# Coloquinte/sleekit

Measured on AMD Instinct MI355X. Metric: Mweights/sec quantized (GPTQ 3-bit, 4096x4096 layer), higher is better.
Workload: dtype f64; 1 GPU; 8 layers 4096x4096, 8-level uniform codebook (GPTQ 3-bit), act_order=diag, damp=0.01, local-search moves=0, layer error included; distinct_inputs=8, allocator_settle_steps=15, gpu_max_hw_queues=4

## Files before the change

sleekit_amd/csrc/api.hip:

```cpp
#include "mfma32.h"
#include "mfma64.h"

namespace slk {

__global__ __launch_bounds__(256) void k_probe_f64(double *sink, int iters) {
    double4_t c0 = {0, 0, 0, 0}, c1 = c0, c2 = c0, c3 = c0;
    const double a = 1.0 + threadIdx.x * 1e-3, b = 1.0 - threadIdx.x * 1e-3;
    for (int i = 0; i < iters; ++i) {
        c0 = __builtin_amdgcn_mfma_f64_16x16x4f64(a, b, c0, 0, 0, 0);
        c1 = __builtin_amdgcn_mfma_f64_16x16x4f64(b, a, c1, 0, 0, 0);
        c2 = __builtin_amdgcn_mfma_f64_16x16x4f64(a, a, c2, 0, 0, 0);
        c3 = __builtin_amdgcn_mfma_f64_16x16x4f64(b, b, c3, 0, 0, 0);
    }
    const double4_t s = c0 + c1 + c2 + c3;
    if (s[0] + s[1] + s[2] + s[3] == 12345.678) sink[0] = s[0];
}

template <int NACC>
__global__ __launch_bounds__(256) void k_probe_f64_n(double *sink, int iters) {
    double4_t c[NACC];
    double a[NACC], b[NACC];
#pragma unroll
    for (int i = 0; i < NACC; ++i) {
        c[i] = (double4_t){0, 0, 0, 0};
// ... 67 lines not shown
}

using namespace slk;

extern "C" {

int slk_probe_chain(double *out, int iters, int mode, slk_stream_t stream) {
    SLK_REQUIRE(out && iters > 0, "bad arguments");
    hipStream_t s = as_stream(stream);
    SLK_RUN("probe_chain", 0, 0, s, k_probe_chain<<<1, 64, 0, s>>>(out, iters, mode));
    return SLK_OK;
}

size_t slk_workspace_bytes(int R, int n) {
    if (R < 0 || n <= 0) return 0;
    const size_t ld = (size_t)slk_factor_ld(n);
    const size_t rn = (size_t)(R > 0 ? R : 1) * (size_t)n;
    size_t factor = 2 * ld * ld * sizeof(double) + 2 * (ld / 64) * sizeof(int);
    size_t loop = 2 * rn * sizeof(float) + (size_t)n * sizeof(int) + 64 * sizeof(float) + 5 * 256;
    size_t search = rn * sizeof(float) + (size_t)(R + n) * sizeof(float) + (size_t)R * ((n + 127) / 128) * sizeof(float) + 4096;
    size_t error = 6 * (rn + 128 * (size_t)n) + 6 * (size_t)n * n + 4 * (size_t)R * ((n + 127) / 128) * sizeof(float) + 8192;
    size_t prep = 64 * sizeof(float) + (size_t)n * (sizeof(double) + 1);
    search += error;
    size_t m = factor;
    if (loop > m) m = loop;
    if (search > m) m = search;
    if (error > m) m = error;
    if (prep > m) m = prep;
    return m + (1u << 16);
}

size_t slk_workspace_bytes_batch(int batch, int rows_per_layer, int n) {
    if (batch < 1 || batch > 64 || rows_per_layer < 0 || n <= 0 || (long long)batch * rows_per_layer > 0x7fffffffLL) return 0;
    return slk_workspace_bytes(batch * rows_per_layer, n) + (size_t)(batch - 1) * 6 * (size_t)n * n +
           (size_t)batch * n * (sizeof(int) + sizeof(float)) + (size_t)(batch - 1) * 64 * sizeof(float) +
           4096;
}

int slk_probe_mfma_f64(double *sink, int blocks, int iters, slk_stream_t stream) {
    SLK_REQUIRE(sink && blocks > 0 && iters > 0, "bad arguments");
    hipStream_t s = as_stream(stream);
    SLK_RUN("probe_mfma_f64", 4.0 * 2048 * 4 * iters * blocks, 0, s, k_probe_f64<<<blocks, 256, 0, s>>>(sink, iters));
    return SLK_OK;
}

int slk_probe_mfma_f64_acc(double *sink, int blocks, int iters, int nacc, slk_stream_t stream) {
    SLK_REQUIRE(sink && blocks > 0 && iters > 0 && (nacc == 1 || nacc == 2 || nacc == 4 || nacc == 8 || nacc == 16), "bad arguments");
    hipStream_t s = as_stream(stream);
    if (nacc == 1)
        SLK_RUN("probe_mfma_f64", 1.0 * 2048 * 4 * iters * blocks, 0, s, k_probe_f64_n<1><<<blocks, 256, 0, s>>>(sink, iters));
    else if (nacc == 2)
        SLK_RUN("probe_mfma_f64", 2.0 * 2048 * 4 * iters * blocks, 0, s, k_probe_f64_n<2><<<blocks, 256, 0, s>>>(sink, iters));
    else if (nacc == 4)
        SLK_RUN("probe_mfma_f64", 4.0 * 2048 * 4 * iters * blocks, 0, s, k_probe_f64_n<4><<<blocks, 256, 0, s>>>(sink, iters));
    else if (nacc == 8)
        SLK_RUN("probe_mfma_f64", 8.0 * 2048 * 4 * iters * blocks, 0, s, k_probe_f64_n<8><<<blocks, 256, 0, s>>>(sink, iters));
    else
        SLK_RUN("probe_mfma_f64", 16.0 * 2048 * 4 * iters * blocks, 0, s, k_probe_f64_n<16><<<blocks, 256, 0, s>>>(sink, iters));
    return SLK_OK;
}

int slk_probe_mfma_f32(float *sink, int blocks, int iters, slk_stream_t stream) {
    SLK_REQUIRE(sink && blocks > 0 && iters > 0, "bad arguments");
    hipStream_t s = as_stream(stream);
    SLK_RUN("probe_mfma_f32", 4.0 * 4096 * 4 * iters * blocks, 0, s, k_probe_f32<<<blocks, 256, 0, s>>>(sink, iters));
    return SLK_OK;
}

}

#include <atomic>
#include <map>
#include <mutex>
#include <string>
#include <vector>
#include <strings.h>

namespace slk {
namespace {
const char *const kOptNames[OPT_COUNT] = {
    "NO_FAST_LEAF", "NO_DEFER", "NO_WINDOW2", "WIN_DBG", "NO_REGULAR_SEARCH", "NO_FAST_SEARCH_DIV",
    "NO_ERROR_SPLITK", "ERROR_CB", "NO_SYM_ERROR", "NO_BF16_ERROR", "NO_BF16_DMA", "NO_BF16_HESSIAN",
    "ERROR_F32_BELOW", "NO_BF16_ASYM", "NO_SYM_AVERAGE", "NO_WAVE_SEARCH", "LOOKAHEAD", "WINDOW_ROWS", "PANEL_SPLIT", "ROWS_BELOW_WIDE",
    "NO_LOOP_ERROR", "CHAIN_CARRIES_BELOW",
};
std::atomic<int> g_opts[OPT_COUNT];
std::once_flag g_opts_once;
void opts_from_env() {
    for (int i = 0; i < OPT_COUNT; ++i) {
        const std::string name = std::string("SLK_") + kOptNames[i];
        const char *v = getenv(name.c_str());
        int val = 0;
        if (v) {
            val = atoi(v);
            if (val == 0 && v[0] != '0') val = 1;
        }
        g_opts[i].store(val, std::memory_order_relaxed);
    }
}
int opt_index(const char *name) {
    if (!name) return -1;
    if (strncasecmp(name, "SLK_", 4) == 0) name += 4;
    for (int i = 0; i < OPT_COUNT; ++i)
        if (strcasecmp(name, kOptNames[i]) == 0) return i;
    return -1;
}
std::mutex g_lds_mu;
std::map<std::pair<const void *, int>, size_t> g_lds_set;
}

int opt(Opt o) {
    std::call_once(g_opts_once, opts_from_env);
    return g_opts[o].load(std::memory_order_relaxed);
}

namespace {
std::mutex g_helper_mu;
struct HelperRec {
    Helper h;
    int made;
};
std::map<std::pair<int, hipStream_t>, HelperRec> g_helpers;
}

hipError_t helper_for(hipStream_t main, int need, Helper *out) {
    if (need > HELPER_EVENTS) return hipErrorInvalidValue;
    int device = 0;
    hipError_t e = hipGetDevice(&device);
    if (e != hipSuccess) return e;
    std::lock_guard<std::mutex> lock(g_helper_mu);
    auto it = g_helpers.find({device, main});
    if (it == g_helpers.end()) {
        HelperRec r{};
        e = hipStreamCreateWithFlags(&r.h.stream, hipStreamNonBlocking);
        if (e != hipSuccess) return e;
        e = hipStreamCreateWithFlags(&r.h.stream2, hipStreamNonBlocking);
        if (e != hipSuccess) {
            (void)hipStreamDestroy(r.h.stream);
            return e;
        }
        r.h.events = new hipEvent_t[HELPER_EVENTS]();
        r.made = 0;
        it = g_helpers.emplace(std::make_pair(device, main), r).first;
    }
    HelperRec &r = it->second;
    const int had = r.made;
    while (r.made < need) {
        e = hipEventCreateWithFlags(&r.h.events[r.made], hipEventDisableTiming);
        if (e != hipSuccess) {
            while (r.made > had) (void)hipEventDestroy(r.h.events[--r.made]);
            if (had == 0) {
                (void)hipStreamDestroy(r.h.stream);
                (void)hipStreamDestroy(r.h.stream2);
                delete[] r.h.events;
                g_helpers.erase(it);
            }
            return e;
        }
        ++r.made;
    }
    *out = r.h;
    return hipSuccess;
}

static hipError_t release_helpers() {
    std::lock_guard<std::mutex> lock(g_helper_mu);
    hipError_t first = hipSuccess;
// ... 156 lines not shown
```

sleekit_amd/csrc/common.h:

```cpp
#pragma once

#include <hip/hip_runtime.h>
#include <stddef.h>
#include <stdint.h>
#include <stdio.h>

#include "../../include/sleekit_amd.h"

namespace slk {

void set_error(const char *fmt, ...);

#define SLK_REQUIRE(cond, ...)          \
    do {                                \
        if (!(cond)) {                  \
            slk::set_error(__VA_ARGS__); \
            return SLK_E_ARG;           \
        }                               \
    } while (0)

#define SLK_HIP(call)                                                                  \
    do {                                                                               \
        hipError_t e_ = (call);                                                        \
        if (e_ != hipSuccess) {                                                        \
            slk::set_error("%s failed: %s (%s:%d)", #call, hipGetErrorString(e_), __FILE__, __LINE__); \
            return SLK_E_HIP;                                                          \
        }                                                                              \
    } while (0)

#define SLK_LAUNCH_CHECK() SLK_HIP(hipGetLastError())

struct ProfScope {
    int slot;
    hipStream_t stream;
    ProfScope(const char *name, double flops, double bytes, hipStream_t s);
    ~ProfScope();
};

void prof_next_width(long workgroups);

#define SLK_RUN(name, flops, bytes, stream, ...)                 \
    do {                                                         \
        {                                                        \
            slk::ProfScope prof_scope_(name, flops, bytes, stream); \
            __VA_ARGS__;                                         \
        }                                                        \
        SLK_LAUNCH_CHECK();                                      \
    } while (0)

#define SLK_RUN_W(name, flops, bytes, wgs, stream, ...) \
    do {                                                \
        slk::prof_next_width((long)(wgs));              \
        SLK_RUN(name, flops, bytes, stream, __VA_ARGS__); \
    } while (0)

enum Opt {
    OPT_NO_FAST_LEAF,
    OPT_NO_DEFER,
    OPT_NO_WINDOW2,
    OPT_WIN_DBG,
    OPT_NO_REGULAR_SEARCH,
    OPT_NO_FAST_SEARCH_DIV,
    OPT_NO_ERROR_SPLITK,
    OPT_ERROR_CB,
    OPT_NO_SYM_ERROR,
    OPT_NO_BF16_ERROR,
    OPT_NO_BF16_DMA,
    OPT_NO_BF16_HESSIAN,
    OPT_ERROR_F32_BELOW,
    OPT_NO_BF16_ASYM,
    OPT_NO_SYM_AVERAGE,
    OPT_NO_WAVE_SEARCH,
    OPT_LOOKAHEAD,
    OPT_WINDOW_ROWS,
    OPT_PANEL_SPLIT,
    OPT_ROWS_BELOW_WIDE,
    OPT_NO_LOOP_ERROR,
    OPT_CHAIN_CARRIES_BELOW,
    OPT_COUNT
};
int opt(Opt o);

struct Helper {
    hipStream_t stream;
    hipStream_t stream2;
    hipEvent_t *events;
};
constexpr int HELPER_EVENTS = 512;
hipError_t helper_for(hipStream_t main, int need, Helper *out);

hipError_t lds_opt_in(const void *kernel, size_t bytes);
#define SLK_LDS_OPT_IN(kernel, bytes) SLK_HIP(slk::lds_opt_in(reinterpret_cast<const void *>(kernel), (bytes)))

struct PtrTable {
    const float *p[64];
};

constexpr int LOOP_LAYERS = 16;
struct LayerTable {
    const float *W[LOOP_LAYERS], *scale[LOOP_LAYERS];
    const long long *order[LOOP_LAYERS];
    const double *U[LOOP_LAYERS];
};
template <class T>
__device__ __forceinline__ const T *layer_base(const T *const (&column)[LOOP_LAYERS], int b, size_t stride) {
    return column[b % LOOP_LAYERS] + (size_t)(b - b % LOOP_LAYERS) * stride;
}

int row_errors_products(const float *W, const float *Q, const float *const *Hs, int batch, int rpl, int n, const int *sym_known,
                        float *row_err, float *G, void *workspace, size_t ws_bytes, slk_stream_t stream);

int loop_error_means(const float *const *Hs, int batch, int n, float *out, hipStream_t s);

static inline hipStream_t as_stream(slk_stream_t s) { return reinterpret_cast<hipStream_t>(s); }

static inline size_t align_up(size_t x, size_t a) { return (x + a - 1) / a * a; }

struct Arena {
    char *base;
    size_t size, used;
    Arena(void *p, size_t bytes) : base(static_cast<char *>(p)), size(bytes), used(0) {}
    template <class T>
    T *take(size_t count) {
        size_t off = align_up(used, 256);
        size_t end = off + count * sizeof(T);
        if (end > size || base == nullptr) return nullptr;
        used = end;
        return reinterpret_cast<T *>(base + off);
    }
};

struct Grid {
    float zero, step, top;
    const float *table;
    int n;
};

static inline Grid make_grid(int levels, double lo, double hi, const float *table = nullptr) {
    Grid g;
    g.zero = (float)lo;
    g.step = (float)((hi - lo) / (double)(levels - 1));
    g.top = (float)(levels - 1);
    g.table = table;
    g.n = levels;
    return g;
}

__device__ __forceinline__ float grid_pos(float x, const Grid g, float shift, float first, float last) {
    float t = (x - g.zero) / g.step;
    t = t + shift;
    t = rintf(t);
    return fminf(fmaxf(t, first), last);
}
__device__ __forceinline__ float grid_val(float t, const Grid g) { return t * g.step + g.zero; }
__device__ __forceinline__ float grid_value(float x, const Grid g) {
    return grid_val(grid_pos(x, g, 0.0f, 0.0f, g.top), g);
}

__device__ __forceinline__ int table_index(float x, const Grid g) {
    const float *lim = g.table + g.n;
    int lo = 0, hi = g.n - 1;
// ... 106 lines not shown
```

sleekit_amd/csrc/factor.hip:

```cpp
#include <stdlib.h>

#include "mfma64.h"

namespace slk {

constexpr int PANEL = 64;
constexpr int OUTER_SMALL = 256, OUTER_LARGE = 512;
constexpr int LOOKAHEAD_MIN_TILES = 24;

__device__ long long g_panel_cycles[16];

constexpr int TP = 66;

struct PanelSmem {
    double t[PANEL][TP];
    double x[PANEL][TP];
    double a21[PANEL][TP];
    double lb[PANEL][TP];
    double rdiag[PANEL];
    int early_count;
};

#ifndef NEWTON_STEPS
#define NEWTON_STEPS 2
// ... 316 lines not shown
        tile64_foreach2(old, acc, [&](int r, int c, double o, double v) { pc[(size_t)r * ld + c] = o - v; });
        return;
    }
    BelowSmem &sm = *reinterpret_cast<BelowSmem *>(smem_raw);
    X += (size_t)blockIdx.z * ld * ld;
    const int lane = t & 63, wave = t >> 6;
    const bool has_prev = kprev >= 0;
    const int sr = t >> 2, sc8 = (t & 3) * 16;
    const int first = (int)blockIdx.x * per_wg, last = min(first + per_wg, tiles_below);
    double vt[16], vb[16];
    auto fetch_tile = [&](int rt) {
        const int r0 = k0 + PANEL * (rt + 1);
        const double *pt = A + (size_t)(r0 + sr) * ld + k0 + sc8;
        load8d<true>(pt, *reinterpret_cast<double(*)[8]>(&vt[0]));
        load8d<true>(pt + 8, *reinterpret_cast<double(*)[8]>(&vt[8]));
        if (has_prev) {
            const double *pl = A + (size_t)(r0 + sr) * ld + kprev + sc8;
            load8d<true>(pl, *reinterpret_cast<double(*)[8]>(&vb[0]));
            load8d<true>(pl + 8, *reinterpret_cast<double(*)[8]>(&vb[8]));
        }
    };
    {
        double vx[16], vk[16];
        const double *px = X + (size_t)(k0 + sr) * ld + k0 + sc8;
        load8d<true>(px, *reinterpret_cast<double(*)[8]>(&vx[0]));
        load8d<true>(px + 8, *reinterpret_cast<double(*)[8]>(&vx[8]));
        if (has_prev) {
            const double *pk = A + (size_t)(k0 + sr) * ld + kprev + sc8;
            load8d<true>(pk, *reinterpret_cast<double(*)[8]>(&vk[0]));
            load8d<true>(pk + 8, *reinterpret_cast<double(*)[8]>(&vk[8]));
        }
        fetch_tile(first);
#pragma unroll
        for (int e = 0; e < 16; e += 2) {
            *reinterpret_cast<double2_t *>(&sm.x[sr][sc8 + e]) = (double2_t){vx[e], vx[e + 1]};
            if (has_prev) *reinterpret_cast<double2_t *>(&sm.lk[sr][sc8 + e]) = (double2_t){vk[e], vk[e + 1]};
        }
    }
    for (int rt = first; rt < last; ++rt) {
        const int r0 = k0 + PANEL * (rt + 1);
#pragma unroll
        for (int e = 0; e < 16; e += 2) {
            *reinterpret_cast<double2_t *>(&sm.a21[sr][sc8 + e]) = (double2_t){vt[e], vt[e + 1]};
            if (has_prev) *reinterpret_cast<double2_t *>(&sm.lb[sr][sc8 + e]) = (double2_t){vb[e], vb[e + 1]};
        }
        __syncthreads();
        if (rt + 1 < last) fetch_tile(rt + 1);
        if (has_prev) {
#pragma unroll
            for (int cb = 0; cb < 4; ++cb) {
                double4_t acc = {0.0, 0.0, 0.0, 0.0};
#pragma unroll
                for (int kq = 0; kq < 4; ++kq) acc = blk_mma_abt(&sm.lb[16 * wave][16 * kq], &sm.lk[16 * cb][16 * kq], acc, 1.0, lane);
                double *cp = &sm.a21[16 * wave][16 * cb];
                double4_t o = blk_load_d(cp, lane);
#pragma unroll
                for (int r = 0; r < 4; ++r) o[r] = o[r] - acc[r];
                blk_store_d(cp, lane, o);
            }
            asm volatile("s_waitcnt lgkmcnt(0)" ::: "memory");
        }
#pragma unroll
        for (int cb = 0; cb < 4; ++cb) {
            double4_t acc = {0.0, 0.0, 0.0, 0.0};
#pragma unroll
            for (int k = 0; k < 4; ++k)
                if (k <= cb) acc = blk_mma_abt(&sm.a21[16 * wave][16 * k], &sm.x[16 * cb][16 * k], acc, 1.0, lane);
#pragma unroll
            for (int r = 0; r < 4; ++r) A[(size_t)(r0 + 16 * wave + (lane >> 4) + 4 * r) * ld + k0 + 16 * cb + (lane & 15)] = acc[r];
        }
        if (rt + 1 < last) __syncthreads();
    }
}


constexpr int INFO_HANDOFF_TIMEOUT = 0x7fffffff;
constexpr bool slk_chain_addressable(int ld) { return (size_t)ld * (size_t)ld * sizeof(double) <= 0xffffffffull; }

typedef unsigned int u32x4_t __attribute__((ext_vector_type(4)));
typedef unsigned int u32x2_t __attribute__((ext_vector_type(2)));
constexpr int AUX_SC1 = 16;
constexpr int CHAIN_CARRY_CAP = 80;
constexpr bool CHAIN_CARRY_BY_RULE = true;

struct GBuf {
    __amdgpu_buffer_rsrc_t rs;
    __device__ __forceinline__ GBuf(const double *base, size_t bytes)
        : rs(__builtin_amdgcn_make_buffer_rsrc(const_cast<double *>(base), 0, (int)(bytes > 0xffffffffull ? 0xffffffffull : bytes), 0x00020000)) {}
    template <int AUX>
    __device__ __forceinline__ double2_t load2(unsigned elem) const {
        const u32x4_t v = __builtin_amdgcn_raw_buffer_load_b128(rs, elem * 8u, 0, AUX);
        return (double2_t){__hiloint2double((int)v[1], (int)v[0]), __hiloint2double((int)v[3], (int)v[2])};
    }
    template <int AUX>
    __device__ __forceinline__ void store2(unsigned elem, double2_t x) const {
        const u32x4_t v = {(unsigned)__double2loint(x[0]), (unsigned)__double2hiint(x[0]), (unsigned)__double2loint(x[1]), (unsigned)__double2hiint(x[1])};
        __builtin_amdgcn_raw_buffer_store_b128(v, rs, elem * 8u, 0, AUX);
    }
};

__device__ __forceinline__ int flag_peek(const int *p) { return __hip_atomic_load(p, __ATOMIC_RELAXED, __HIP_MEMORY_SCOPE_AGENT); }
__device__ __forceinline__ bool flag_wait(const int *p, int want) {
    bool ok = flag_peek(p) >= want;
    if (!ok) {
        const unsigned long long t0 = __builtin_amdgcn_s_memrealtime();
        for (;;) {
            __builtin_amdgcn_s_sleep(1);
            if (flag_peek(p) >= want) {
                ok = true;
                break;
            }
            if (__builtin_amdgcn_s_memrealtime() - t0 > 200000000ull) break;
        }
    }
    __builtin_amdgcn_fence(__ATOMIC_ACQUIRE, "wavefront");
    return ok;
}
__device__ __forceinline__ void flag_publish(int *p, int value) {
    asm volatile("s_waitcnt vmcnt(0)" ::: "memory");
    __syncthreads();
    if (threadIdx.x == 0) __hip_atomic_store(p, value, __ATOMIC_RELAXED, __HIP_MEMORY_SCOPE_AGENT);
}

struct TileRegs {
    double2_t v[8];
};
template <int AUX, int J0 = 0, int J1 = 8>
__device__ __forceinline__ void tile_fetch(TileRegs &r, const GBuf &g, unsigned elem0, int ld) {
    const int t = threadIdx.x;
#pragma unroll
    for (int j = J0; j < J1; ++j) r.v[j] = g.load2<AUX>(elem0 + (unsigned)(8 * j + (t >> 5)) * (unsigned)ld + 2u * (t & 31));
}
template <int J0 = 0, int J1 = 8>
__device__ __forceinline__ void tile_stash(double (*img)[TP], const TileRegs &r) {
    const int t = threadIdx.x;
#pragma unroll
    for (int j = J0; j < J1; ++j) *reinterpret_cast<double2_t *>(&img[8 * j + (t >> 5)][2 * (t & 31)]) = r.v[j];
}
template <int AUX, int J0 = 0, int J1 = 8>
__device__ __forceinline__ void tile_store_from_lds(const GBuf &g, unsigned elem0, int ld, const double (*img)[TP]) {
    const int t = threadIdx.x;
#pragma unroll
    for (int j = J0; j < J1; ++j)
        g.store2<AUX>(elem0 + (unsigned)(8 * j + (t >> 5)) * (unsigned)ld + 2u * (t & 31), *reinterpret_cast<const double2_t *>(&img[8 * j + (t >> 5)][2 * (t & 31)]));
}

template <class Early>
__device__ __forceinline__ int diag_tile_factor(PanelSmem &sm, int lane, int wave, Early rows_0_and_1_are_in) {
    auto diag_inverse = [&](int kb) {
        const int c0 = 16 * kb, c = lane & 15;
        double xv[16];
#pragma unroll
        for (int i = 0; i < 16; ++i) {
            double s = 0.0;
#pragma unroll
            for (int u = 0; u < i; ++u) s = __builtin_fma(sm.t[c0 + i][c0 + u], xv[u], s);
            xv[i] = ((c == i ? 1.0 : 0.0) - s) * sm.rdiag[c0 + i];
        }
        if (lane < 16) {
#pragma unroll
            for (int i = 0; i < 16; ++i) sm.x[c0 + i][c0 + c] = xv[i];
        }
    };
    auto block_owner = [](int rb, int cb) { return cb == 1 ? rb : (rb == 3 && cb == 2 ? 2 : 1); };
    auto block_update = [&](int rb, int cb, int kb) {
        double *c = &sm.t[16 * rb][16 * cb];
// ... 309 lines not shown
    auto tile_elem = [&](int tr, int tc) { return (unsigned)(K0 + PANEL * tr) * (unsigned)ld + (unsigned)(K0 + PANEL * tc); };
    auto load_c = [&](int q) {
        const double *p = A + (size_t)(rows0 + (lane >> 4)) * ld + K0 + PANEL * q + 16 * wave + (lane & 15);
        return (double4_t){p[0], p[(size_t)4 * ld], p[(size_t)8 * ld], p[(size_t)12 * ld]};
    };
    TileRegs nx;
    tile_fetch<0>(nx, gx, tile_elem(0, 0), ld);
    double4_t c = load_c(0), cnext = load_c(nb > 1 ? 1 : 0);
    for (int q = 0; q < nb; ++q) {
        for (int s = 0; s <= q; ++s) {
            const bool tri = s == q;
            __syncthreads();
            tile_stash(sm.bt, nx);
            if (tri) blk_store_d(&sm.c[0][16 * wave], lane, c);
            __syncthreads();
            if (!tri) {
                if (s + 1 < q) tile_fetch<0>(nx, ga, tile_elem(q, s + 1), ld);
                else tile_fetch<0>(nx, gx, tile_elem(q, q), ld);
            } else if (q + 1 < nb) {
                tile_fetch<0>(nx, ga, tile_elem(q + 1, 0), ld);
            }
            if (!tri) {
                double4_t acc = {0.0, 0.0, 0.0, 0.0};
#pragma unroll
                for (int kq = 0; kq < 4; ++kq) acc = blk_mma_abt(&sm.own[s][0][16 * kq], &sm.bt[16 * wave][16 * kq], acc, 1.0, lane);
                c = c - acc;
            } else {
                double4_t acc = {0.0, 0.0, 0.0, 0.0};
#pragma unroll
                for (int k = 0; k < 4; ++k)
                    if (k <= wave) acc = blk_mma_abt(&sm.c[0][16 * k], &sm.bt[16 * wave][16 * k], acc, 1.0, lane);
#pragma unroll
                for (int j = 0; j < 4; ++j) A[(size_t)(rows0 + (lane >> 4) + 4 * j) * ld + K0 + PANEL * q + 16 * wave + (lane & 15)] = acc[j];
                blk_store_d(&sm.own[q][0][16 * wave], lane, acc);
                c = cnext;
                if (q + 2 < nb) cnext = load_c(q + 2);
            }
        }
    }
}

__global__ __launch_bounds__(256) void k_syrk_tiles(double *__restrict__ A, int ld, int ti0, int tj0, int ka,
                                                    int kb) {
    __shared__ __attribute__((aligned(16))) Tile64Smem sm;
    A += (size_t)blockIdx.z * ld * ld;
    const int bi = ti0 + blockIdx.y, bj = tj0 + blockIdx.x;
    if (bj > bi) return;
    Acc64 acc;
    acc.zero();
    const int t = threadIdx.x;
    const double *pa = A + ((size_t)bi * TILE + (t >> 2)) * ld + (t & 3) * 8;
    const double *pb = A + ((size_t)bj * TILE + (t >> 2)) * ld + (t & 3) * 8;
    double *pc = A + (size_t)bi * TILE * ld + (size_t)bj * TILE;
    Acc64 old;
    tile64_map(old, [&](int r, int c) { return pc[(size_t)r * ld + c]; });
    tile64_mac<false>(
        acc, sm, ka, kb, [&](int k0, double(&v)[8]) { load8d<true>(pa + k0, v); },
        [&](int k0, double(&v)[8]) { load8d<true>(pb + k0, v); });
    tile64_foreach2(old, acc, [&](int r, int c, double o, double v) { pc[(size_t)r * ld + c] = o - v; });
}

__global__ __launch_bounds__(256) void k_syrk_triangle(double *__restrict__ A, int ld, int t0, int m, int ka, int kb) {
    __shared__ __attribute__((aligned(16))) Tile64Smem sm;
    A += (size_t)blockIdx.z * ld * ld;
    const int total = m * (m + 1) / 2, per_xcd = (total + 7) / 8;
    const int lin = (blockIdx.x & 7) * per_xcd + (blockIdx.x >> 3);
    if (lin >= total) return;
    int row = (int)((sqrtf(8.0f * (float)lin + 1.0f) - 1.0f) * 0.5f);
    while (row * (row + 1) / 2 > lin) --row;
    while ((row + 1) * (row + 2) / 2 <= lin) ++row;
    const int bi = t0 + row, bj = t0 + lin - row * (row + 1) / 2;
    Acc64 acc;
    acc.zero();
    const int t = threadIdx.x;
    const double *pa = A + ((size_t)bi * TILE + (t >> 2)) * ld + (t & 3) * 8;
    const double *pb = A + ((size_t)bj * TILE + (t >> 2)) * ld + (t & 3) * 8;
    tile64_mac<false>(
        acc, sm, ka, kb, [&](int k0, double(&v)[8]) { load8d<true>(pa + k0, v); },
        [&](int k0, double(&v)[8]) { load8d<true>(pb + k0, v); });
    double *pc = A + (size_t)bi * TILE * ld + (size_t)bj * TILE;
    Acc64 old;
    tile64_map(old, [&](int r, int c) { return pc[(size_t)r * ld + c]; });
    tile64_foreach2(old, acc, [&](int r, int c, double o, double v) { pc[(size_t)r * ld + c] = o - v; });
}

template <int STAGE>
__global__ __launch_bounds__(256) void k_trtri_level(const double *__restrict__ L, double *__restrict__ X,
                                                     double *__restrict__ S, int ld, int nt, int s, int node0) {
    __shared__ __attribute__((aligned(16))) Tile64Smem sm;
    L += (size_t)blockIdx.z * ld * ld;
    X += (size_t)blockIdx.z * ld * ld;
    S += (size_t)blockIdx.z * ld * ld;
    const int id = blockIdx.x;
    const int per_node = s * s, node = node0 + id / per_node, in_node = id % per_node;
    const int deep = in_node / s, other = in_node % s;
    const int lo = node * 2 * s, mid = lo + s;
    const int bi = (STAGE == 0) ? mid + other : mid + (s - 1 - deep);
    const int bj = (STAGE == 0) ? lo + deep : lo + other;
    if (bi >= nt) return;
    Acc64 acc;
    acc.zero();
    const int t = threadIdx.x;
    if (STAGE == 0) {
        const double *pa = L + ((size_t)bi * TILE + (t >> 2)) * ld + (t & 3) * 8;
        const double *pb = X + (size_t)(t >> 3) * ld + (size_t)bj * TILE + (t & 7) * 2;
        tile64_mac<true>(
            acc, sm, bj * TILE, mid * TILE, [&](int k0, double(&v)[8]) { load8d<true>(pa + k0, v); },
            [&](int k0, double(&v)[8]) { load8d_cols(pb + (size_t)k0 * ld, v); });
        double *pc = S + (size_t)bi * TILE * ld + (size_t)bj * TILE;
        tile64_foreach(acc, [&](int r, int c, double v) { pc[(size_t)r * ld + c] = v; });
    } else {
        const double *pa = X + ((size_t)bi * TILE + (t >> 2)) * ld + (t & 3) * 8;
        const double *pb = S + (size_t)(t >> 3) * ld + (size_t)bj * TILE + (t & 7) * 2;
        tile64_mac<true>(
            acc, sm, mid * TILE, (bi + 1) * TILE, [&](int k0, double(&v)[8]) { load8d<true>(pa + k0, v); },
            [&](int k0, double(&v)[8]) { load8d_cols(pb + (size_t)k0 * ld, v); });
        double *pc = X + (size_t)bi * TILE * ld + (size_t)bj * TILE;
        tile64_foreach(acc, [&](int r, int c, double v) { pc[(size_t)r * ld + c] = -v; });
    }
}

__global__ __launch_bounds__(256) void k_flip_out(const double *__restrict__ X, int ld, int n,
                                                  double *__restrict__ U) {
    X += (size_t)blockIdx.z * ld * ld;
    U += (size_t)blockIdx.z * n * n;
    for (int i = blockIdx.x; i < n; i += gridDim.x) {
        const double *src = X + (size_t)(n - 1 - i) * ld;
        double *dst = U + (size_t)i * n;
        for (int j = threadIdx.x; j < n; j += blockDim.x) dst[j] = (j >= i) ? src[n - 1 - j] : 0.0;
    }
}

__global__ void k_clear_info(int *info, int *flags, int per_matrix) {
    if (threadIdx.x == 0) info[blockIdx.x] = 0;
    if (flags)
        for (int i = threadIdx.x; i < per_matrix; i += blockDim.x) flags[(size_t)blockIdx.x * per_matrix + i] = 0;
}

}

using namespace slk;

static int chol_inverse_impl(double *A, int batch, int n, double *U, int *info, void *workspace, size_t ws_bytes,
                             slk_stream_t stream, bool want_lookahead) {
    const int ld = slk_factor_ld(n);
    const int nt = ld / TILE;
    const unsigned B = (unsigned)batch;
    const double Bd = (double)batch;
    Arena ws(workspace, ws_bytes);
    double *X = ws.take<double>((size_t)ld * ld * batch);
    double *S = ws.take<double>((size_t)ld * ld * batch);
    int *flags = ws.take<int>((size_t)batch * 2 * nt);
    if (!X || !S || !flags) {
        set_error("workspace too small for %d factorisation(s) of %d x %d", batch, n, n);
        return SLK_E_WS;
    }
    hipStream_t s = as_stream(stream);
    const int OUTER = n >= 4096 ? OUTER_LARGE : OUTER_SMALL;
    SLK_LDS_OPT_IN(k_chol_panel, sizeof(PanelSmem));
    SLK_RUN_W("clear_info", 0, 4, 1, s, k_clear_info<<<B, 64, 0, s>>>(info, flags, 2 * nt));

    Helper helper{};
    const bool lookahead = (want_lookahead || opt(OPT_LOOKAHEAD)) && nt >= LOOKAHEAD_MIN_TILES + OUTER / TILE && nt / (OUTER / TILE) < HELPER_EVENTS / 3;
    if (lookahead) SLK_HIP(helper_for(s, 3 * (nt / (OUTER / TILE) + 1), &helper));
    const int sp = opt(OPT_PANEL_SPLIT);
    const bool chain = (sp == 0 || sp == 3) && slk_chain_addressable(ld);
    const bool split = !chain && !want_lookahead && sp != 2 && (sp == 1 || batch > 1 || n >= 8192);
    if (split) SLK_LDS_OPT_IN(k_panel_below, sizeof(BelowSmem));
    if (chain) {
        SLK_LDS_OPT_IN(k_chol_chain<false>, sizeof(PanelSmem));
        SLK_LDS_OPT_IN(k_chol_chain<true>, sizeof(PanelSmem));
        SLK_LDS_OPT_IN(k_chol_chain_below, sizeof(PanelSmem));
        SLK_LDS_OPT_IN(k_chol_rows_below, sizeof(RowsBelowSmem));
    }
    int inv_done[2][16] = {{0}, {0}};
    auto inverse_nodes = [&](int tiles_done, hipStream_t st) -> int {
        int li = 0;
        for (int lvl = 1; lvl < nt; lvl *= 2, ++li) {
            const int all = (nt + 2 * lvl - 1) / (2 * lvl);
            for (int stage = 0; stage < 2; ++stage) {
                int ready;
                if (tiles_done >= nt) ready = all;
                else if (stage == 0) ready = tiles_done >= lvl ? (tiles_done - lvl) / (2 * lvl) + 1 : 0;
                else ready = tiles_done / (2 * lvl);
                if (ready > all) ready = all;
                const int first = inv_done[stage][li], count = ready - first;
                if (count <= 0) continue;
                inv_done[stage][li] = ready;
                double fl = 0, tiles = 0;
                for (int nd = first; nd < ready; ++nd) {
                    const int lo = nd * 2 * lvl, mid = lo + lvl, hi = lo + 2 * lvl < nt ? lo + 2 * lvl : nt;
                    for (int bi = mid; bi < hi; ++bi)
                        for (int bj = lo; bj < mid; ++bj) {
                            fl += 2.0 * 64 * 64 * 64 * (stage == 0 ? mid - bj : bi + 1 - mid);
                            tiles += 1;
                        }
                }
                if (tiles == 0) continue;
                dim3 grid(count * lvl * lvl, 1, B);
                if (stage == 0)
                    SLK_RUN_W("trtri_stage0", Bd * fl, Bd * (fl / 64 * 8.0 / 2 + tiles * 8.0 * 64 * 64), tiles * batch, st,
                              k_trtri_level<0><<<grid, 256, 0, st>>>(A, X, S, ld, nt, lvl, first));
                else
                    SLK_RUN_W("trtri_stage1", Bd * fl, Bd * (fl / 64 * 8.0 / 2 + tiles * 8.0 * 64 * 64), tiles * batch, st,
                              k_trtri_level<1><<<grid, 256, 0, st>>>(A, X, S, ld, nt, lvl, first));
            }
        }
        return SLK_OK;
    };
    const int EV = chain ? 3 : 2;
    int block = 0, forked = -1;
    int inverse_on_helper = -1;
    for (int K0 = 0; K0 < ld; K0 += OUTER) {
        const int K1 = K0 + OUTER < ld ? K0 + OUTER : ld;
        if (chain) {
            const int nb = (K1 - K0) / PANEL;
            int below_tiles = (ld - K1) / PANEL;
            const double e = 64.0 * nb;
            const int cc = opt(OPT_CHAIN_CARRIES_BELOW);
            const bool carry = below_tiles > 0 && !lookahead && opt(OPT_ROWS_BELOW_WIDE) == 0 && (nb + below_tiles) * batch <= CHAIN_CARRY_CAP &&
                               (cc == 1 || (cc == 0 && CHAIN_CARRY_BY_RULE));
            if (carry) {
                SLK_RUN_W("chol_chain", Bd * (e * e * e / 3.0 + 64.0 * below_tiles * e * e), Bd * (12.0 * e * e + 16.0 * 64 * below_tiles * e + 4.0 * e * e),
                          (nb + below_tiles) * batch, s,
                          k_chol_chain_below<<<dim3(nb + below_tiles, 1, B), 256, sizeof(PanelSmem), s>>>(A, ld, K0, nb, X, info, flags, opt(OPT_WIN_DBG) & 8));
                below_tiles = 0;
            } else
                SLK_RUN_W("chol_chain", Bd * e * e * e / 3.0, Bd * 12.0 * e * e, nb * batch, s,
                          k_chol_chain<false><<<dim3(nb, 1, B), 256, sizeof(PanelSmem), s>>>(A, ld, K0, nb, X, info, flags, opt(OPT_WIN_DBG) & 8));
            if (below_tiles > 0 && forked >= 0) {
                SLK_HIP(hipStreamWaitEvent(s, helper.events[EV * forked + 1], 0));
                forked = -1;
            }
            const int rw = opt(OPT_ROWS_BELOW_WIDE);
            const bool wide = rw == 1 || (rw == 0 && 4 * below_tiles * batch >= 1024);
            if (below_tiles > 0 && wide)
                SLK_RUN_W("chol_rows_below", Bd * 64.0 * below_tiles * e * e, Bd * (16.0 * 64 * below_tiles * e + 4.0 * e * e), below_tiles * batch, s,
                          k_chol_chain<true><<<dim3(below_tiles, 1, B), 256, sizeof(PanelSmem), s>>>(A, ld, K0, nb, X, info, flags, 0));
            else if (below_tiles > 0)
                SLK_RUN_W("chol_rows_below", Bd * 64.0 * below_tiles * e * e, Bd * (16.0 * 64 * below_tiles * e + 4.0 * e * e), 4 * below_tiles * batch, s,
                          k_chol_rows_below<<<dim3(4 * below_tiles, 1, B), 256, sizeof(RowsBelowSmem), s>>>(A, ld, K0, nb, X));
        }
        for (int k0 = K0; k0 < K1 && !chain; k0 += PANEL) {
            const int below = (ld - k0) / PANEL;
            const int kprev = k0 > K0 ? k0 - PANEL : -1;
            const int rest_cols = kprev >= 0 ? (K1 - k0) / PANEL - 1 : 0;
            int rest = 0;
            for (int c = 0; c < rest_cols; ++c) rest += nt - (k0 / TILE + 1 + c);
            const double prologue = kprev >= 0 ? (double)below * 2.0 * 64 * 64 * 64 + (double)below * 2.0 * 64 * 64 * 64 : 0.0;
            if (split) {
                const double pro1 = kprev >= 0 ? 2.0 * 64 * 64 * 64 : 0.0;
                SLK_RUN_W("chol_panel", Bd * (2.0 / 3.0 * 64 * 64 * 64 + pro1), Bd * 16.0 * 64 * 64, batch, s,
                          k_chol_panel<<<dim3(1, 1, B), 256, sizeof(PanelSmem), s>>>(A, ld, k0, kprev, 1, 0, X, info, opt(OPT_WIN_DBG) & 8));
                if (below - 1 + rest > 0) {
                    const int per_wg = 2;
                    const int nbw = (below - 1 + per_wg - 1) / per_wg;
                    SLK_RUN_W("chol_panel_below",
                              Bd * ((double)(below - 1) * 64 * 64 * 64 + (kprev >= 0 ? (double)(below - 1) * 2.0 * 64 * 64 * 64 : 0.0) +
                                    (double)rest * 2.0 * 64 * 64 * PANEL),
                              Bd * (24.0 * (below - 1) * 64 * 64 + (double)rest * 16.0 * 64 * 64), (nbw + rest) * batch, s,
                              k_panel_below<<<dim3(nbw + rest, 1, B), 256, sizeof(BelowSmem), s>>>(A, ld, k0, kprev, nbw, rest_cols, X, below - 1,
                                                                                                  per_wg));
                }
            } else {
                SLK_RUN_W("chol_panel",
                          Bd * (2.0 / 3.0 * 64 * 64 * 64 + (double)(below - 1) * 64 * 64 * 64 + prologue + (double)rest * 2.0 * 64 * 64 * PANEL),
                          Bd * (16.0 * below * 64 * 64 + (double)rest * 16.0 * 64 * 64), (below + rest) * batch, s,
                          k_chol_panel<<<dim3(below + rest, 1, B), 256, sizeof(PanelSmem), s>>>(A, ld, k0, kprev, below, rest_cols, X, info,
                                                                                                opt(OPT_WIN_DBG) & 8));
            }
        }
        const int t0 = K1 / TILE;
        if (nt > t0) {
            const int m = nt - t0, total = m * (m + 1) / 2;
            const double tiles = total;
            const int ahead = OUTER / TILE;
            if (lookahead && chain && m >= LOOKAHEAD_MIN_TILES) {
                SLK_HIP(hipEventRecord(helper.events[EV * block], s));
                const int nbn = ahead < m ? ahead : m, td = nbn * (nbn + 1) / 2;
                SLK_RUN_W("chol_syrk_ahead", Bd * td * 2.0 * 64 * 64 * (K1 - K0), Bd * (16.0 * nbn * 64 * (K1 - K0) + td * 16.0 * 64 * 64), td * batch, s,
                          k_syrk_tiles<<<dim3(nbn, nbn, B), 256, 0, s>>>(A, ld, t0, t0, K0, K1));
                SLK_HIP(hipStreamWaitEvent(helper.stream, helper.events[EV * block], 0));
                const int m2 = m - nbn, total2 = m2 * (m2 + 1) / 2;
                if (m2 > 0) {
                    SLK_RUN_W("chol_syrk_outer", Bd * (double)nbn * m2 * 2.0 * 64 * 64 * (K1 - K0), Bd * (8.0 * (ld - K1) * (K1 - K0) + (double)nbn * m2 * 16.0 * 64 * 64),
                              (double)nbn * m2 * batch, helper.stream,
                              k_syrk_tiles<<<dim3(nbn, m2, B), 256, 0, helper.stream>>>(A, ld, t0 + nbn, t0, K0, K1));
                    SLK_RUN_W("chol_syrk_outer", Bd * total2 * 2.0 * 64 * 64 * (K1 - K0), Bd * (8.0 * (ld - K1) * (K1 - K0) + total2 * 16.0 * 64 * 64),
                              (double)total2 * batch, helper.stream,
                              k_syrk_triangle<<<dim3(8 * ((total2 + 7) / 8), 1, B), 256, 0, helper.stream>>>(A, ld, t0 + nbn, m2, K0, K1));
                }
                SLK_HIP(hipEventRecord(helper.events[EV * block + 1], helper.stream));
                forked = block;
                SLK_HIP(hipStreamWaitEvent(helper.stream2, helper.events[EV * block], 0));
                {
                    const int rc = inverse_nodes(t0, helper.stream2);
                    if (rc != SLK_OK) return rc;
                }
                SLK_HIP(hipEventRecord(helper.events[EV * block + 2], helper.stream2));
                inverse_on_helper = block;
            } else if (lookahead && m >= LOOKAHEAD_MIN_TILES) {
                if (block > 0) SLK_HIP(hipStreamWaitEvent(s, helper.events[2 * (block - 1) + 1], 0));
                SLK_HIP(hipEventRecord(helper.events[2 * block], s));
                const double ta = (double)ahead * m - 6;
                SLK_RUN_W("chol_syrk_ahead", Bd * ta * 2.0 * 64 * 64 * (K1 - K0), Bd * (8.0 * (ld - K1) * (K1 - K0) + ta * 16.0 * 64 * 64),
                          ta * batch, s, k_syrk_tiles<<<dim3(ahead, m, B), 256, 0, s>>>(A, ld, t0, t0, K0, K1));
                SLK_HIP(hipStreamWaitEvent(helper.stream, helper.events[2 * block], 0));
                const int m2 = m - ahead, total2 = m2 * (m2 + 1) / 2;
                SLK_RUN_W("chol_syrk_outer", Bd * total2 * 2.0 * 64 * 64 * (K1 - K0), Bd * (8.0 * (ld - K1) * (K1 - K0) + total2 * 16.0 * 64 * 64),
                          (double)total2 * batch, helper.stream,
                          k_syrk_triangle<<<dim3(8 * ((total2 + 7) / 8), 1, B), 256, 0, helper.stream>>>(A, ld, t0 + ahead, m2, K0, K1));
                SLK_HIP(hipEventRecord(helper.events[2 * block + 1], helper.stream));
                forked = block;
            } else {
                if (forked >= 0) {
                    SLK_HIP(hipStreamWaitEvent(s, helper.events[EV * forked + 1], 0));
                    forked = -1;
                }
                if (lookahead && chain) {
                    SLK_HIP(hipEventRecord(helper.events[EV * block], s));
                    SLK_HIP(hipStreamWaitEvent(helper.stream2, helper.events[EV * block], 0));
                    const int rc = inverse_nodes(t0, helper.stream2);
                    if (rc != SLK_OK) return rc;
                    SLK_HIP(hipEventRecord(helper.events[EV * block + 2], helper.stream2));
                    inverse_on_helper = block;
                }
                SLK_RUN_W("chol_syrk_outer", Bd * tiles * 2.0 * 64 * 64 * (K1 - K0), Bd * (8.0 * (ld - K1) * (K1 - K0) + tiles * 16.0 * 64 * 64),
                          tiles * batch, s, k_syrk_triangle<<<dim3(8 * ((total + 7) / 8), 1, B), 256, 0, s>>>(A, ld, t0, m, K0, K1));
            }
        }
        ++block;
    }
    if (forked >= 0) SLK_HIP(hipStreamWaitEvent(s, helper.events[EV * forked + 1], 0));
    if (inverse_on_helper >= 0) SLK_HIP(hipStreamWaitEvent(s, helper.events[EV * inverse_on_helper + 2], 0));
    {
        const int rc = inverse_nodes(nt, s);
        if (rc != SLK_OK) return rc;
    }
    SLK_RUN("flip_out", 0, Bd * 12.0 * n * n, s, k_flip_out<<<dim3(n < 2048 ? n : 2048, 1, B), 256, 0, s>>>(X, ld, n, U));
    return SLK_OK;
}

extern "C" int slk_chol_inverse_upper(double *A, int n, double *U, int *info, void *workspace,
                                      size_t ws_bytes, slk_stream_t stream) {
    SLK_REQUIRE(A && U && info && n > 0, "bad arguments");
    return chol_inverse_impl(A, 1, n, U, info, workspace, ws_bytes, stream, false);
}

extern "C" int slk_chol_inverse_upper_lookahead(double *A, int n, double *U, int *info, void *workspace,
                                                size_t ws_bytes, slk_stream_t stream) {
    SLK_REQUIRE(A && U && info && n > 0, "bad arguments");
    return chol_inverse_impl(A, 1, n, U, info, workspace, ws_bytes, stream, true);
}

extern "C" int slk_chol_inverse_upper_batch(double *A, int batch, int n, double *U, int *info, void *workspace,
                                            size_t ws_bytes, slk_stream_t stream) {
    SLK_REQUIRE(A && U && info && n > 0, "bad arguments");
    SLK_REQUIRE(batch >= 1 && batch <= 64, "batch must be 1..64");
    return chol_inverse_impl(A, batch, n, U, info, workspace, ws_bytes, stream, false);
}

extern "C" int slk_probe_panel_cycles(long long *host_out, int reset) {
    SLK_REQUIRE(host_out, "null pointer");
    SLK_HIP(hipDeviceSynchronize());
    SLK_HIP(hipMemcpyFromSymbol(host_out, HIP_SYMBOL(g_panel_cycles), sizeof(long long) * 16));
    if (reset) {
        long long zero[16] = {0};
        SLK_HIP(hipMemcpyToSymbol(HIP_SYMBOL(g_panel_cycles), zero, sizeof(zero)));
    }
    return SLK_OK;
}

extern "C" size_t slk_factor_workspace_bytes_batch(int batch, int n) {
    if (batch < 1 || batch > 64 || n <= 0) return 0;
    const size_t ld = (size_t)slk_factor_ld(n);
    return 2 * ld * ld * sizeof(double) * batch + (size_t)batch * (64 * sizeof(float) + (size_t)n * (sizeof(double) + sizeof(int))) +
           (size_t)batch * 2 * (ld / 64) * sizeof(int) + (1u << 16);
}
```

sleekit_amd/csrc/mfma64.h:

```cpp
#pragma once

#include <type_traits>

#include "common.h"

namespace slk {

typedef double double4_t __attribute__((ext_vector_type(4)));
typedef double double2_t __attribute__((ext_vector_type(2)));
typedef float float4v_t __attribute__((ext_vector_type(4)));

constexpr int TILE = 64;
constexpr int KSTEP = 32;
constexpr int PITCH_RK = 34;
constexpr int PITCH_KC = 80;

struct Tile64Smem {
    double a[TILE * PITCH_RK];
    double b[KSTEP * PITCH_KC];
};

constexpr int PITCH_AF = 36;
struct Tile64SmemAf {
    float a[TILE * PITCH_AF];
// ... 86 lines not shown
template <bool B_C_FAST, class TA = double, class SM, class LA, class LB>
__device__ __forceinline__ void tile64_mac(Acc64 &acc, SM &sm, int k_begin, int k_end, LA la, LB lb) {
    constexpr bool AF = std::is_same<SM, Tile64SmemAf>::value;
    static_assert(!AF || (std::is_same<TA, float>::value && B_C_FAST), "the float32 A image is for float32 A and column-contiguous B");
    using TL = typename std::conditional<AF, float, double>::type;
    constexpr int PITCH_A = AF ? PITCH_AF : PITCH_RK;
    const int t = threadIdx.x;
    const int lane = t & 63, wave = t >> 6;
    const int wr = wave >> 1, wc = wave & 1;
    TA ra[8];
    double rb[8];
    TL *a_dst = sm.a + (t >> 2) * PITCH_A + (t & 3) * 8;
    double *b_dst = B_C_FAST ? sm.b + (t >> 3) * PITCH_KC + (t & 7) * 2 : sm.b + (t >> 2) * PITCH_RK + (t & 3) * 8;
    constexpr int B_PIECE = B_C_FAST ? 16 : 2;

    auto stash = [&]() {
        if constexpr (AF) {
#pragma unroll
            for (int h = 0; h < 2; ++h)
                *reinterpret_cast<float4v_t *>(a_dst + 4 * h) = (float4v_t){(float)ra[4 * h], (float)ra[4 * h + 1], (float)ra[4 * h + 2], (float)ra[4 * h + 3]};
        }
#pragma unroll
        for (int h = 0; h < 4; ++h) {
            if constexpr (!AF) *reinterpret_cast<double2_t *>(a_dst + 2 * h) = (double2_t){(double)ra[2 * h], (double)ra[2 * h + 1]};
            *reinterpret_cast<double2_t *>(b_dst + B_PIECE * h) = (double2_t){rb[2 * h], rb[2 * h + 1]};
        }
    };

    if (k_begin >= k_end) return;
    la(k_begin, ra);
    lb(k_begin, rb);
    const TL *a_src = sm.a + (wr * 32 + (lane & 15)) * PITCH_A + (lane >> 4);
    const double *b_src = B_C_FAST ? sm.b + (lane >> 4) * PITCH_KC + wc * 32 + (lane & 15)
                                   : sm.b + (wc * 32 + (lane & 15)) * PITCH_RK + (lane >> 4);
    int a_off1 = 16 * PITCH_A, b_off1 = B_C_FAST ? 16 : 16 * PITCH_RK;
    asm volatile("" : "+v"(a_off1), "+v"(b_off1));
    const TL *a_src1 = a_src + a_off1;
    const double *b_src1 = b_src + b_off1;
    for (int k0 = k_begin; k0 < k_end; k0 += KSTEP) {
#ifdef SLK_T64_NO_STAGE
        if (k0 == k_begin) {
            __syncthreads();
            stash();
            __syncthreads();
        }
#else
        __syncthreads();
        stash();
        __syncthreads();
        if (k0 + KSTEP < k_end) {
            la(k0 + KSTEP, ra);
            lb(k0 + KSTEP, rb);
        }
#endif
#ifdef SLK_T64_NO_READS
        TL a0n = 1.0, a1n = 2.0;
        double b0n = 3.0, b1n = 4.0;
        asm volatile("" : "+v"(a0n), "+v"(a1n), "+v"(b0n), "+v"(b1n));
#else
        TL a0n = a_src[0], a1n = a_src1[0];
        double b0n = b_src[0], b1n = b_src1[0];
#endif
        asm volatile("" ::: "memory");
#pragma unroll
        for (int kk = 0; kk < KSTEP; kk += 4) {
            const double a0 = (double)a0n, a1 = (double)a1n, b0 = b0n, b1 = b1n;
#ifndef SLK_T64_NO_READS
            if (kk + 4 < KSTEP) {
                a0n = a_src[kk + 4];
                a1n = a_src1[kk + 4];
                b0n = B_C_FAST ? b_src[(kk + 4) * PITCH_KC] : b_src[kk + 4];
                b1n = B_C_FAST ? b_src1[(kk + 4) * PITCH_KC] : b_src1[kk + 4];
            }
#endif
            asm volatile("" : "+v"(acc.c[0][0]), "+v"(acc.c[0][1])::"memory");
            acc.c[0][0] = __builtin_amdgcn_mfma_f64_16x16x4f64(a0, b0, acc.c[0][0], 0, 0, 0);
            acc.c[0][1] = __builtin_amdgcn_mfma_f64_16x16x4f64(a0, b1, acc.c[0][1], 0, 0, 0);
            acc.c[1][0] = __builtin_amdgcn_mfma_f64_16x16x4f64(a1, b0, acc.c[1][0], 0, 0, 0);
            acc.c[1][1] = __builtin_amdgcn_mfma_f64_16x16x4f64(a1, b1, acc.c[1][1], 0, 0, 0);
        }
    }
}


template <class F>
__device__ __forceinline__ void tile64_foreach(const Acc64 &acc, F f) {
    const int lane = threadIdx.x & 63, wave = threadIdx.x >> 6;
    const int wr = wave >> 1, wc = wave & 1;
#pragma unroll
    for (int i = 0; i < 2; ++i)
#pragma unroll
        for (int j = 0; j < 2; ++j)
#pragma unroll
            for (int r = 0; r < 4; ++r)
                f(wr * 32 + i * 16 + (lane >> 4) + 4 * r, wc * 32 + j * 16 + (lane & 15), acc.c[i][j][r]);
}

template <class F>
__device__ __forceinline__ void tile64_map(Acc64 &acc, F value) {
    const int lane = threadIdx.x & 63, wave = threadIdx.x >> 6;
    const int wr = wave >> 1, wc = wave & 1;
#pragma unroll
    for (int i = 0; i < 2; ++i)
#pragma unroll
        for (int j = 0; j < 2; ++j)
#pragma unroll
            for (int r = 0; r < 4; ++r) acc.c[i][j][r] = value(wr * 32 + i * 16 + (lane >> 4) + 4 * r, wc * 32 + j * 16 + (lane & 15));
}
template <class F>
__device__ __forceinline__ void tile64_foreach2(const Acc64 &x, const Acc64 &y, F f) {
    const int lane = threadIdx.x & 63, wave = threadIdx.x >> 6;
    const int wr = wave >> 1, wc = wave & 1;
#pragma unroll
    for (int i = 0; i < 2; ++i)
#pragma unroll
        for (int j = 0; j < 2; ++j)
#pragma unroll
            for (int r = 0; r < 4; ++r)
                f(wr * 32 + i * 16 + (lane >> 4) + 4 * r, wc * 32 + j * 16 + (lane & 15), x.c[i][j][r], y.c[i][j][r]);
}

}
```

Baseline: 6535 Mweights/s.

## Split small SYRK and TRTRI tile launches into 32x32 quadrant workgroups

Adds quadrant variants of the Cholesky trailing SYRK update and the blocked triangular-inverse level kernels. Each 64x64 output tile is split across four 256-thread workgroups computing 32x32 sub-tiles with a new tile32 MFMA helper. The quadrant path is used when the workgroup count falls below a threshold, and env options can force it on or off. The goal is more parallelism for small launches that underfill the GPU, at the cost of reloading A and B panels twice and lower per-workgroup arithmetic intensity.

New measurement: 6593 Mweights/s, median of 6. Within noise of the previous version (+0.9%).

```diff
diff --git a/sleekit_amd/csrc/api.hip b/sleekit_amd/csrc/api.hip
--- a/sleekit_amd/csrc/api.hip
+++ b/sleekit_amd/csrc/api.hip
@@ -173,7 +173,7 @@
     "NO_FAST_LEAF", "NO_DEFER", "NO_WINDOW2", "WIN_DBG", "NO_REGULAR_SEARCH", "NO_FAST_SEARCH_DIV",
     "NO_ERROR_SPLITK", "ERROR_CB", "NO_SYM_ERROR", "NO_BF16_ERROR", "NO_BF16_DMA", "NO_BF16_HESSIAN",
     "ERROR_F32_BELOW", "NO_BF16_ASYM", "NO_SYM_AVERAGE", "NO_WAVE_SEARCH", "LOOKAHEAD", "WINDOW_ROWS", "PANEL_SPLIT", "ROWS_BELOW_WIDE",
-    "NO_LOOP_ERROR", "CHAIN_CARRIES_BELOW",
+    "NO_LOOP_ERROR", "CHAIN_CARRIES_BELOW", "SYRK_QUADRANTS", "TRTRI_QUADRANTS",
 };
 std::atomic<int> g_opts[OPT_COUNT];
 std::once_flag g_opts_once;
diff --git a/sleekit_amd/csrc/common.h b/sleekit_amd/csrc/common.h
--- a/sleekit_amd/csrc/common.h
+++ b/sleekit_amd/csrc/common.h
@@ -77,6 +77,8 @@
     OPT_ROWS_BELOW_WIDE,
     OPT_NO_LOOP_ERROR,
     OPT_CHAIN_CARRIES_BELOW,
+    OPT_SYRK_QUADRANTS,
+    OPT_TRTRI_QUADRANTS,
     OPT_COUNT
 };
 int opt(Opt o);
diff --git a/sleekit_amd/csrc/factor.hip b/sleekit_amd/csrc/factor.hip
--- a/sleekit_amd/csrc/factor.hip
+++ b/sleekit_amd/csrc/factor.hip
@@ -422,6 +422,8 @@
 constexpr int AUX_SC1 = 16;
 constexpr int CHAIN_CARRY_CAP = 80;
 constexpr bool CHAIN_CARRY_BY_RULE = true;
+constexpr int SYRK_QUADRANTS_BELOW = 400;
+constexpr int TRTRI_QUADRANTS_BELOW = 300;
 
 struct GBuf {
     __amdgpu_buffer_rsrc_t rs;
@@ -897,6 +899,31 @@
     Acc64 old;
     tile64_map(old, [&](int r, int c) { return pc[(size_t)r * ld + c]; });
     tile64_foreach2(old, acc, [&](int r, int c, double o, double v) { pc[(size_t)r * ld + c] = o - v; });
+}
+
+__global__ __launch_bounds__(256) void k_syrk_triangle_quadrants(double *__restrict__ A, int ld, int t0, int m, int ka, int kb) {
+    __shared__ __attribute__((aligned(16))) Tile32Smem sm;
+    A += (size_t)blockIdx.z * ld * ld;
+    const int total = 4 * (m * (m + 1) / 2), per_xcd = (total + 7) / 8;
+    const int lin4 = (blockIdx.x & 7) * per_xcd + (blockIdx.x >> 3);
+    if (lin4 >= total) return;
+    const int lin = lin4 >> 2, qr = (lin4 >> 1) & 1, qc = lin4 & 1;
+    int row = (int)((sqrtf(8.0f * (float)lin + 1.0f) - 1.0f) * 0.5f);
+    while (row * (row + 1) / 2 > lin) --row;
+    while ((row + 1) * (row + 2) / 2 <= lin) ++row;
+    const int bi = t0 + row, bj = t0 + lin - row * (row + 1) / 2;
+    const int t = threadIdx.x, lane = t & 63, wave = t >> 6;
+    const double *pa = A + ((size_t)bi * TILE + 32 * qr + (t >> 3)) * ld + (t & 7) * 4;
+    const double *pb = A + ((size_t)bj * TILE + 32 * qc + (t >> 3)) * ld + (t & 7) * 4;
+    double *pc = A + ((size_t)bi * TILE + 32 * qr + 16 * (wave >> 1) + (lane >> 4)) * ld + (size_t)bj * TILE + 32 * qc + 16 * (wave & 1) + (lane & 15);
+    double old[4];
+#pragma unroll
+    for (int r = 0; r < 4; ++r) old[r] = pc[(size_t)(4 * r) * ld];
+    double4_t acc = {0.0, 0.0, 0.0, 0.0};
+    tile32_mac<false>(
+        acc, sm, ka, kb, [&](int k0, double(&v)[4]) { load4d(pa + k0, v); }, [&](int k0, double(&v)[4]) { load4d(pb + k0, v); });
+#pragma unroll
+    for (int r = 0; r < 4; ++r) pc[(size_t)(4 * r) * ld] = old[r] - acc[r];
 }
 
 template <int STAGE>
@@ -935,6 +962,34 @@
     }
 }
 
+template <int STAGE>
+__global__ __launch_bounds__(256) void k_trtri_level_quadrants(const double *__restrict__ L, double *__restrict__ X,
+                                                               double *__restrict__ S, int ld, int nt, int s, int node0) {
+    __shared__ __attribute__((aligned(16))) Tile32Smem sm;
+    L += (size_t)blockIdx.z * ld * ld;
+    X += (size_t)blockIdx.z * ld * ld;
+    S += (size_t)blockIdx.z * ld * ld;
+    const int id = blockIdx.x >> 2, qr = (blockIdx.x >> 1) & 1, qc = blockIdx.x & 1;
+    const int per_node = s * s, node = node0 + id / per_node, in_node = id % per_node;
+    const int deep = in_node / s, other = in_node % s;
+    const int lo = node * 2 * s, mid = lo + s;
+    const int bi = (STAGE == 0) ? mid + other : mid + (s - 1 - deep);
+    const int bj = (STAGE == 0) ? lo + deep : lo + other;
+    if (bi >= nt) return;
+    const int t = threadIdx.x, lane = t & 63, wave = t >> 6;
+    double4_t acc = {0.0, 0.0, 0.0, 0.0};
+    const double *A0 = (STAGE == 0) ? L : X, *B0 = (STAGE == 0) ? X : S;
+    const double *pa = A0 + ((size_t)bi * TILE + 32 * qr + (t >> 3)) * ld + (t & 7) * 4;
+    const double *pb = B0 + (size_t)(t >> 3) * ld + (size_t)bj * TILE + 32 * qc + (t & 7) * 4;
+    const int ka = (STAGE == 0) ? bj * TILE : mid * TILE, kb = (STAGE == 0) ? mid * TILE : (bi + 1) * TILE;
+    tile32_mac<true>(
+        acc, sm, ka, kb, [&](int k0, double(&v)[4]) { load4d(pa + k0, v); }, [&](int k0, double(&v)[4]) { load4d(pb + (size_t)k0 * ld, v); });
+    double *pc = ((STAGE == 0) ? S : X) + ((size_t)bi * TILE + 32 * qr + 16 * (wave >> 1) + (lane >> 4)) * ld + (size_t)bj * TILE + 32 * qc +
+                 16 * (wave & 1) + (lane & 15);
+#pragma unroll
+    for (int r = 0; r < 4; ++r) pc[(size_t)(4 * r) * ld] = (STAGE == 0) ? acc[r] : -acc[r];
+}
+
 __global__ __launch_bounds__(256) void k_flip_out(const double *__restrict__ X, int ld, int n,
                                                   double *__restrict__ U) {
     X += (size_t)blockIdx.z * ld * ld;
@@ -1013,6 +1068,19 @@
                 }
                 if (tiles == 0) continue;
                 dim3 grid(count * lvl * lvl, 1, B);
+                const int tq = opt(OPT_TRTRI_QUADRANTS);
+                const long wgs = (long)count * lvl * lvl * batch;
+                const bool quadrants = tq == 1 || (tq != 2 && wgs < (tq > 2 ? tq : TRTRI_QUADRANTS_BELOW));
+                if (quadrants) {
+                    dim3 grid4(4 * count * lvl * lvl, 1, B);
+                    if (stage == 0)
+                        SLK_RUN_W("trtri_level", Bd * fl, Bd * (fl / 64 * 8.0 + tiles * 8.0 * 64 * 64), 4 * tiles * batch, st,
+                                  k_trtri_level_quadrants<0><<<grid4, 256, 0, st>>>(A, X, S, ld, nt, lvl, first));
+                    else
+                        SLK_RUN_W("trtri_level", Bd * fl, Bd * (fl / 64 * 8.0 + tiles * 8.0 * 64 * 64), 4 * tiles * batch, st,
+                                  k_trtri_level_quadrants<1><<<grid4, 256, 0, st>>>(A, X, S, ld, nt, lvl, first));
+                    continue;
+                }
                 if (stage == 0)
                     SLK_RUN_W("trtri_stage0", Bd * fl, Bd * (fl / 64 * 8.0 / 2 + tiles * 8.0 * 64 * 64), tiles * batch, st,
                               k_trtri_level<0><<<grid, 256, 0, st>>>(A, X, S, ld, nt, lvl, first));
@@ -1140,8 +1208,14 @@
                     SLK_HIP(hipEventRecord(helper.events[EV * block + 2], helper.stream2));
                     inverse_on_helper = block;
                 }
-                SLK_RUN_W("chol_syrk_outer", Bd * tiles * 2.0 * 64 * 64 * (K1 - K0), Bd * (8.0 * (ld - K1) * (K1 - K0) + tiles * 16.0 * 64 * 64),
-                          tiles * batch, s, k_syrk_triangle<<<dim3(8 * ((total + 7) / 8), 1, B), 256, 0, s>>>(A, ld, t0, m, K0, K1));
+                const int sq = opt(OPT_SYRK_QUADRANTS);
+                const bool quadrants = sq == 1 || (sq != 2 && (long)total * batch < (sq > 2 ? sq : SYRK_QUADRANTS_BELOW));
+                if (quadrants)
+                    SLK_RUN_W("chol_syrk_quadrants", Bd * tiles * 2.0 * 64 * 64 * (K1 - K0), Bd * (2 * 8.0 * (ld - K1) * (K1 - K0) + tiles * 16.0 * 64 * 64),
+                              4 * tiles * batch, s, k_syrk_triangle_quadrants<<<dim3(8 * ((4 * total + 7) / 8), 1, B), 256, 0, s>>>(A, ld, t0, m, K0, K1));
+                else
+                    SLK_RUN_W("chol_syrk_outer", Bd * tiles * 2.0 * 64 * 64 * (K1 - K0), Bd * (8.0 * (ld - K1) * (K1 - K0) + tiles * 16.0 * 64 * 64),
+                              tiles * batch, s, k_syrk_triangle<<<dim3(8 * ((total + 7) / 8), 1, B), 256, 0, s>>>(A, ld, t0, m, K0, K1));
             }
         }
         ++block;
diff --git a/sleekit_amd/csrc/mfma64.h b/sleekit_amd/csrc/mfma64.h
--- a/sleekit_amd/csrc/mfma64.h
+++ b/sleekit_amd/csrc/mfma64.h
@@ -192,6 +192,57 @@
     }
 }
 
+constexpr int PITCH_KC32 = 48;
+struct Tile32Smem {
+    double a[32 * PITCH_RK];
+    double b[KSTEP * PITCH_KC32];
+};
+
+template <bool B_C_FAST, class LA, class LB>
+__device__ __forceinline__ void tile32_mac(double4_t &acc, Tile32Smem &sm, int k_begin, int k_end, LA la, LB lb) {
+    const int t = threadIdx.x;
+    const int lane = t & 63, wave = t >> 6;
+    const int wr = wave >> 1, wc = wave & 1;
+    double ra[4], rb[4];
+    double *a_dst = sm.a + (t >> 3) * PITCH_RK + (t & 7) * 4;
+    double *b_dst = sm.b + (t >> 3) * (B_C_FAST ? PITCH_KC32 : PITCH_RK) + (t & 7) * 4;
+    if (k_begin >= k_end) return;
+    la(k_begin, ra);
+    lb(k_begin, rb);
+    const double *a_src = sm.a + (wr * 16 + (lane & 15)) * PITCH_RK + (lane >> 4);
+    const double *b_src = B_C_FAST ? sm.b + (lane >> 4) * PITCH_KC32 + wc * 16 + (lane & 15) : sm.b + (wc * 16 + (lane & 15)) * PITCH_RK + (lane >> 4);
+    for (int k0 = k_begin; k0 < k_end; k0 += KSTEP) {
+        __syncthreads();
+#pragma unroll
+        for (int h = 0; h < 2; ++h) {
+            *reinterpret_cast<double2_t *>(a_dst + 2 * h) = (double2_t){ra[2 * h], ra[2 * h + 1]};
+            *reinterpret_cast<double2_t *>(b_dst + 2 * h) = (double2_t){rb[2 * h], rb[2 * h + 1]};
+        }
+        __syncthreads();
+        if (k0 + KSTEP < k_end) {
+            la(k0 + KSTEP, ra);
+            lb(k0 + KSTEP, rb);
+        }
+        double a[KSTEP / 4], b[KSTEP / 4];
+#pragma unroll
+        for (int g = 0; g < KSTEP / 4; ++g) {
+            a[g] = a_src[4 * g];
+            b[g] = B_C_FAST ? b_src[4 * g * PITCH_KC32] : b_src[4 * g];
+        }
+#pragma unroll
+        for (int g = 0; g < KSTEP / 4; ++g) acc = __builtin_amdgcn_mfma_f64_16x16x4f64(a[g], b[g], acc, 0, 0, 0);
+    }
+}
+
+__device__ __forceinline__ void load4d(const double *p, double (&v)[4]) {
+#pragma unroll
+    for (int h = 0; h < 2; ++h) {
+        const double2_t x = *reinterpret_cast<const double2_t *>(p + 2 * h);
+        v[2 * h] = x[0];
+        v[2 * h + 1] = x[1];
+    }
+}
+
 
 template <class F>
 __device__ __forceinline__ void tile64_foreach(const Acc64 &acc, F f) {
```
